# NTT123/vietTTS

Hardware: NVIDIA H100
Metric: audio_samples_per_sec (higher is better)
Workload: dtype f32 (bf16x3 split products on wgmma tensor cores, fp32 accumulate/storage)

## Files before the change

viettts_b200/csrc/tc_conv.cu:

```cuda
#include <cuda_bf16.h>

#include <algorithm>

#include "tc_common.cuh"
#include "vtts_internal.cuh"

namespace {

using namespace tcx;

constexpr int NCWG = 2;
constexpr int NCONS = NCWG * 128;
constexpr int PROD_WARP = NCONS / 32;
constexpr int NCONV = 96;
constexpr int NTHREADS = NCONS + 32 + NCONV;
constexpr int NA = 4;
constexpr int HALO = 64;
constexpr int PAIR_OVERLAP = 16;
constexpr int NQ = 2;
constexpr int NREADERS = (NCONS + NCONV) / 32;

template <int N, int MW, int PAIRF, bool STAGED = false>
struct TcCfg {
  static constexpr int R = 64 * MW * NCWG;
  static constexpr int R_OUT = R - PAIR_OVERLAP;
  static constexpr int RA = R + HALO;
  static constexpr int A_STAGE = RA * 64;
  static constexpr int W_STAGE = N * 64;
  static constexpr int NW = N == 256 ? 4 : 8;
  static constexpr int NCH2 = PAIRF ? N / 16 : 0;
  static constexpr int EPI_NC = N < 128 ? N : 128;
  static constexpr int EPI_LD = EPI_NC + 8;
  static constexpr int EPI_WG = 64 * EPI_LD + N;
  static constexpr int EPI_STAGE = STAGED ? NCWG * EPI_WG * 4 : 0;
  static constexpr int SMEM_BYTES =
      NA * A_STAGE + NW * W_STAGE + NCH2 * A_STAGE + EPI_STAGE + (2 * NA + 2 * NW + 2 * NQ) * 8 + NQ * 4 + 1024;
  static_assert(SMEM_BYTES <= 227 * 1024, "shared memory of one CTA");
};

struct Ring {
  uint32_t s = 0, p = 0;
  template <int NS>
  __device__ __forceinline__ void next() { if (++s == NS) { s = 0; p ^= 1; } }
};

struct Tile {
  int pi, b, tt, ph;
};
__device__ __forceinline__ Tile decode_tile(int t, int nph, int nprob, int tiles_per_row) {
  Tile d;
  d.ph = t % nph; t /= nph;
  d.pi = t % nprob; t /= nprob;
  d.tt = t % tiles_per_row;
  d.b = t / tiles_per_row;
  return d;
}

__device__ __forceinline__ int take_ticket(int* sched, int ntiles) {
  const int t = (int)gridDim.x + atomicAdd(&sched[0], 1);
  if (t < ntiles) return t;
  __threadfence();
  if (atomicAdd(&sched[1], 1) == (int)gridDim.x - 1) {
    atomicExch(&sched[0], 0);
    atomicExch(&sched[1], 0);
  }
  return -1;
}

struct TileQueue {
  int* id;
  uint64_t* full;
  uint64_t* empty;
  Ring r;
  __device__ __forceinline__ void put(int t, int* err, long long& acc) {
    mbar_wait_t(&empty[r.s], r.p ^ 1, err, 6, acc);
    id[r.s] = t;
    mbar_arrive(&full[r.s]);
    r.next<NQ>();
  }
  __device__ __forceinline__ int get(int* err, long long& acc) {
    int t = 0;
    if ((threadIdx.x & 31) == 0) {
      mbar_wait_t(&full[r.s], r.p, err, 6, acc);
      t = id[r.s];
      mbar_arrive(&empty[r.s]);
    }
    r.next<NQ>();
    return __shfl_sync(0xffffffffu, t, 0);
  }
};

template <int RA, bool F16>
__device__ __forceinline__ void convert_chunk(uint8_t* stage, int ct, const float* x0, const float* x1, const float* x2, int ld, int c,
                                              int row_base, int rows, int lo, int valid, int pre_mode, float slope) {
  constexpr int RSTEP = NCONV / 4;
  const int q = ct & 3;
  const int r0 = ct >> 2;
  uint8_t* st = stage + ((q >> 1) * RA) * 16 + (q & 1) * 8;
  const int coff = c * 16 + q * 4;
  constexpr int U = 8;
  for (int rr0 = r0; rr0 < rows; rr0 += RSTEP * U) {
    float4 v[U];
#pragma unroll
    for (int u = 0; u < U; ++u) {
      const int rr = rr0 + u * RSTEP;
      const int t = row_base + rr;
      v[u] = make_float4(0.f, 0.f, 0.f, 0.f);
      if (rr < rows && t >= lo && t < valid) {
        const size_t off = (size_t)t * ld + coff;
        v[u] = ldg_pf256(x0 + off);
        if (pre_mode == 2) {
          const float4 a = ldg_pf256(x1 + off);
          const float4 bb = ldg_pf256(x2 + off);
          v[u].x = ((v[u].x + a.x) + bb.x) / 3.0f;
          v[u].y = ((v[u].y + a.y) + bb.y) / 3.0f;
          v[u].z = ((v[u].z + a.z) + bb.z) / 3.0f;
          v[u].w = ((v[u].w + a.w) + bb.w) / 3.0f;
        }
      }
    }
#pragma unroll
    for (int u = 0; u < U; ++u) {
      const int rr = rr0 + u * RSTEP;
      if (rr < rows) {
        float4 x = v[u];
        if (pre_mode >= 1) {
          x.x = lrelu(x.x, slope); x.y = lrelu(x.y, slope); x.z = lrelu(x.z, slope); x.w = lrelu(x.w, slope);
        }
        if constexpr (F16) {
          *reinterpret_cast<uint2*>(st + (size_t)rr * 16) = f16x4_sat(x);
        } else {
          uint2 hi, lo;
          split4(x, hi, lo);
          *reinterpret_cast<uint2*>(st + (size_t)rr * 16) = hi;
          *reinterpret_cast<uint2*>(st + (size_t)(2 * RA + rr) * 16) = lo;
        }
      }
    }
  }
}

template <int N, int NW, bool F16>
__device__ __forceinline__ void produce_weights(uint8_t* w_st, uint64_t* w_full, uint64_t* w_empty, Ring& rw, const void* wpk, int nch,
                                                int k, int* err, long long& wait_acc) {
  constexpr int WB = F16 ? N * 32 : N * 64;
  const uint8_t* src = reinterpret_cast<const uint8_t*>(wpk);
  for (int i = 0; i < nch * k; ++i) {
    mbar_wait_t(&w_empty[rw.s], rw.p ^ 1, err, 4, wait_acc);
    mbar_expect_tx(&w_full[rw.s], WB);
    bulk_g2s(w_st + rw.s * (N * 64), src + (size_t)i * WB, WB, &w_full[rw.s]);
    rw.next<NW>();
  }
}

template <int N, int MW, int RA, int NW, bool A_FROM_RING, bool A_REGS, bool F16>
__device__ __forceinline__ void consume(float (&acc)[MW][N / 2], int wg, uint32_t a_st_u32, uint64_t* a_full, uint64_t* a_empty, Ring& ra,
                                        uint32_t w_st_u32, uint64_t* w_full, uint64_t* w_empty, Ring& rw, int nch, int k, int dil,
                                        int* err, long long& w_a, long long& w_w) {
  const uint64_t a_tmpl = make_desc(0, RA * 16, 128);
  const uint64_t b_tmpl = make_desc(0, (F16 ? 1 : 2) * N * 16, 128);
  const bool lane0 = (threadIdx.x & 31) == 0;
  int pend_w = -1, pend_a = -1;
  for (int c = 0; c < nch; ++c) {
    uint32_t a_base;
    if constexpr (A_FROM_RING) {
      mbar_wait_t(&a_full[ra.s], ra.p, err, 2, w_a);
      a_base = a_st_u32 + ra.s * (RA * 64);
    } else {
      a_base = a_st_u32 + c * (RA * 64);
    }
    for (int j = 0; j < k; ++j) {
      mbar_wait_t(&w_full[rw.s], rw.p, err, 3, w_w);
      const uint32_t w_base = w_st_u32 + rw.s * (N * 64);
      const uint64_t b_hi = b_tmpl | (uint64_t)(w_base >> 4);
      const uint64_t b_lo = b_tmpl | (uint64_t)((w_base + N * 16) >> 4);
      const uint32_t first = (c | j) != 0 ? 1u : 0u;
      if constexpr (A_REGS) {
        static_assert(!A_FROM_RING && !F16, "register A operand: bf16 planes of the fixed buffer");
        const int lane = threadIdx.x & 31, wl = (threadIdx.x >> 5) & 3;
        uint32_t fa_hi[MW][4], fa_lo[MW][4];
#pragma unroll
        for (int mt = 0; mt < MW; ++mt) {
          const int row = (wg * MW + mt) * 64 + wl * 16 + ((lane >> 3) & 1) * 8 + (lane & 7) + j * dil;
          const uint32_t addr = a_base + ((lane >> 4) * RA + row) * 16;
          ldmatrix_x4(fa_hi[mt], addr);
          ldmatrix_x4(fa_lo[mt], addr + 2 * RA * 16);
        }
        wgmma_fence();
#pragma unroll
        for (int mt = 0; mt < MW; ++mt) {
          wgmma_rs<N>(acc[mt], fa_hi[mt], b_hi, first);
          wgmma_rs<N>(acc[mt], fa_hi[mt], b_lo, 1u);
          wgmma_rs<N>(acc[mt], fa_lo[mt], b_hi, 1u);
        }
        wgmma_commit();
        wgmma_wait<0>();
        if (lane == 0) mbar_arrive(&w_empty[rw.s]);
        rw.next<NW>();
        continue;
      }
      wgmma_fence();
#pragma unroll
      for (int mt = 0; mt < MW; ++mt) {
        const uint32_t row = a_base + ((wg * MW + mt) * 64 + j * dil) * 16;
        const uint64_t a_hi = a_tmpl | (uint64_t)(row >> 4);
        const uint64_t a_lo = a_tmpl | (uint64_t)((row + 2 * RA * 16) >> 4);
        if constexpr (F16) {
          wgmma<N, true>(acc[mt], a_hi, b_hi, first);
        } else {
          wgmma<N>(acc[mt], a_hi, b_hi, first);
          wgmma<N>(acc[mt], a_hi, b_lo, 1u);
          wgmma<N>(acc[mt], a_lo, b_hi, 1u);
        }
      }
      wgmma_commit();
      wgmma_wait<1>();
      if (lane0) {
        if (pend_w >= 0) mbar_arrive(&w_empty[pend_w]);
        if (pend_a >= 0) mbar_arrive(&a_empty[pend_a]);
      }
      pend_w = (int)rw.s;
      pend_a = (A_FROM_RING && j == k - 1) ? (int)ra.s : -1;
      rw.next<NW>();
    }
    if constexpr (A_FROM_RING) ra.next<NA>();
  }
  wgmma_wait<0>();
  if (lane0) {
    if (pend_w >= 0) mbar_arrive(&w_empty[pend_w]);
    if (pend_a >= 0) mbar_arrive(&a_empty[pend_a]);
  }
}

__device__ __forceinline__ void cp_async16(void* smem_dst, const void* gsrc) {
  asm volatile("cp.async.cg.shared.global [%0], [%1], 16;" ::"r"(smem_u32(smem_dst)), "l"(gsrc) : "memory");
}
__device__ __forceinline__ void cp_async_commit() { asm volatile("cp.async.commit_group;" ::: "memory"); }
__device__ __forceinline__ void cp_async_wait_all() { asm volatile("cp.async.wait_all;" ::: "memory"); }

__device__ __forceinline__ void init_barriers(uint64_t* bars, int nw) {
  uint64_t* a_full = bars;
  uint64_t* a_empty = bars + NA;
  uint64_t* w_full = bars + 2 * NA;
  uint64_t* w_empty = bars + 2 * NA + nw;
  uint64_t* q_full = bars + 2 * NA + 2 * nw;
  uint64_t* q_empty = q_full + NQ;
  for (int i = 0; i < NA; ++i) { mbar_init(&a_full[i], NCONV); mbar_init(&a_empty[i], NCONS / 32); }
  for (int i = 0; i < nw; ++i) { mbar_init(&w_full[i], 1); mbar_init(&w_empty[i], NCONS / 32); }
  for (int i = 0; i < NQ; ++i) { mbar_init(&q_full[i], 1); mbar_init(&q_empty[i], NREADERS); }
  asm volatile("fence.mbarrier_init.release.cluster;" ::: "memory");
}

__device__ __forceinline__ TileQueue tile_queue(uint64_t* bars, int nw) {
  uint64_t* q_full = bars + 2 * NA + 2 * nw;
  return TileQueue{reinterpret_cast<int*>(q_full + 2 * NQ), q_full, q_full + NQ, Ring{}};
}

#define PRODUCER_TILES                                                                     \
  TileQueue q = tile_queue(bars, NW);                                                      \
  long long w_q = 0;                                                                       \
  int t_next = blockIdx.x;                                                                 \
  q.put(t_next, L.err, w_q);                                                               \
  auto next_tile = [&]() {                                                                 \
    const int t = t_next;                                                                  \
    if (t >= 0) { t_next = take_ticket(L.sched, L.ntiles); q.put(t_next, L.err, w_q); }    \
    return t;                                                                              \
  };
#define READER_TILES                                                                       \
  TileQueue q = tile_queue(bars, NW);                                                      \
  long long w_q = 0;                                                                       \
  auto next_tile = [&]() { return q.get(L.err, w_q); };

template <int N, int EPI, int MW, bool F16>
__global__ void __launch_bounds__(NTHREADS, 1) tc_conv_kernel(const __grid_constant__ TcLaunch L) {
  using Cfg = TcCfg<N, MW, 0, EPI == 0>;
  constexpr int R = Cfg::R, RA = Cfg::RA, NW = Cfg::NW;
  extern __shared__ uint8_t smem_raw[];
  uint8_t* smem = (uint8_t*)(((uintptr_t)smem_raw + 1023) & ~(uintptr_t)1023);
  uint8_t* a_st = smem;
  uint8_t* w_st = smem + NA * Cfg::A_STAGE;
  float* epi_st = reinterpret_cast<float*>(smem_raw + (w_st + NW * Cfg::W_STAGE - smem_raw));
  uint64_t* bars = reinterpret_cast<uint64_t*>(w_st + NW * Cfg::W_STAGE + Cfg::EPI_STAGE);
  uint64_t* a_full = bars;
  uint64_t* a_empty = bars + NA;
  uint64_t* w_full = bars + 2 * NA;
  uint64_t* w_empty = bars + 2 * NA + NW;

  const int tid = threadIdx.x;
  const int warp = __shfl_sync(0xffffffffu, tid >> 5, 0);
  if (tid == 0) init_barriers(bars, NW);
  __syncthreads();

  const int nch = L.Cin / 16;
  const int nph = L.nphase > 1 ? L.nphase : 1;

  constexpr bool ROW_BOUNDS = EPI == 0;
#define TILE_LOOP_BEGIN                                                           \
  for (int tile; (tile = next_tile()) >= 0;) {                                    \
    const Tile td = decode_tile(tile, nph, L.nprob, L.tiles_per_row);              \
    const int ph = td.ph, b = td.b;                                                 \
    const int tau0 = td.tt * R;                                                    \
    const TcProb& P = L.p[td.pi];                                                  \
    int valid = L.T_rows, in_lo = 0, out_hi = 0;                                  \
    if (ROW_BOUNDS && P.rb) {                                                     \
      in_lo = P.rb[3 * b]; valid = P.rb[3 * b + 1]; out_hi = P.rb[3 * b + 2];     \
      if (tau0 * P.out_stride + P.out_off_ph[ph] >= out_hi) continue;             \
    } else {                                                                      \
      if (L.len) {                                                                \
        const int v = L.len[b] * L.len_mul;                                       \
        valid = v < valid ? v : valid;                                            \
      }                                                                           \
      if (tau0 >= valid) continue;                                                \
    }
#define TILE_LOOP_END }

  if (warp == PROD_WARP) {
    if ((tid & 31) == 0) {
      Ring rw;
      long long w_e = 0;
      PRODUCER_TILES
      TILE_LOOP_BEGIN
        (void)b; (void)tau0; (void)in_lo; (void)valid; (void)out_hi;
        produce_weights<N, NW, F16>(w_st, w_full, w_empty, rw, P.wpk_ph[ph], nch, P.k, L.err, w_e);
      TILE_LOOP_END
      if (L.dbg) L.dbg[(size_t)blockIdx.x * 16 + 4] = w_e;
    }
  } else if (warp > PROD_WARP) {
    const int ct = tid - NCONS - 32;
    Ring ra;
    long long w_ae = 0;
    READER_TILES
    TILE_LOOP_BEGIN
      const int k = P.k, dil = P.dil;
      const size_t in_base = (size_t)b * L.T_rows * L.in_ld;
      const float* x1 = L.pre_mode == 2 ? P.x1 + in_base : nullptr;
      const float* x2 = L.pre_mode == 2 ? P.x2 + in_base : nullptr;
      for (int c = 0; c < nch; ++c) {
        mbar_wait_t(&a_empty[ra.s], ra.p ^ 1, L.err, 5, w_ae);
        convert_chunk<RA, F16>(a_st + ra.s * Cfg::A_STAGE, ct, P.x0 + in_base, x1, x2, L.in_ld, c, tau0 + P.in_off_ph[ph], R + (k - 1) * dil,
                          in_lo, valid, L.pre_mode, L.pre_slope);
        fence_proxy_async();
        mbar_arrive(&a_full[ra.s]);
        ra.next<NA>();
      }
      (void)out_hi;
    TILE_LOOP_END
    if (L.dbg && ct == 0) L.dbg[(size_t)blockIdx.x * 16 + 5] = w_ae;
  } else {
    const int wg = warp >> 2, lane = tid & 31;
    float acc[MW][N / 2];
    Ring ra, rw;
    long long w_a = 0, w_w = 0, t_epi = 0;
    const long long t_begin = clock64();
    const int n_valid = (EPI && L.n_valid > 0) ? L.n_valid : N;
    const int post_act = EPI ? L.post_act : 0;
    constexpr int EPI_NC = Cfg::EPI_NC, EPI_LD = Cfg::EPI_LD, RPS = 128 / (EPI_NC / 4), NQ4 = 64 / RPS;
    float* stg = epi_st + wg * Cfg::EPI_WG;
    float* stg_bias = stg + 64 * EPI_LD;
    const int fr = (warp & 3) * 16 + (lane >> 2), fc = 2 * (lane & 3);
    const int dr = (tid & 127) / (EPI_NC / 4), dq = (tid & 127) % (EPI_NC / 4);
    READER_TILES
    TILE_LOOP_BEGIN
      const size_t out_base = (size_t)b * L.rows_out * L.out_ld;
      const int ostride = P.out_stride, ooff = P.out_off_ph[ph];
      auto row_ok = [&](int tau) { return (ROW_BOUNDS && P.rb) ? tau * ostride + ooff < out_hi : tau < valid; };
      auto fetch_pass = [&](int mt, int nh) {
        if (P.resid) {
          const int blk = tau0 + (wg * MW + mt) * 64;
#pragma unroll
          for (int i = 0; i < NQ4; ++i) {
            const int row = i * RPS + dr, tau = blk + row;
            if (row_ok(tau))
              cp_async16(stg + row * EPI_LD + dq * 4, P.resid + out_base + ((tau * ostride + ooff) * L.out_ld + nh * EPI_NC + dq * 4));
          }
        }
        cp_async_commit();
      };
      auto wait_pass = [&]() {
        cp_async_wait_all();
        named_bar(2 + wg, 128);
      };
      if constexpr (EPI == 0) {
        if ((tid & 127) < N / 4) cp_async16(stg_bias + (tid & 127) * 4, P.bias + (tid & 127) * 4);
        fetch_pass(0, 0);
      }
      consume<N, MW, RA, NW, true, false, F16>(acc, wg, smem_u32(a_st), a_full, a_empty, ra, smem_u32(w_st), w_full, w_empty, rw, nch, P.k,
                                               P.dil, L.err, w_a, w_w);
      const long long t_epi0 = clock64();
      if constexpr (EPI == 0) {
        wait_pass();
#pragma unroll
        for (int mt = 0; mt < MW; ++mt) {
          if (!row_ok(tau0 + (wg * MW + mt) * 64)) break;
#pragma unroll
          for (int nh = 0; nh < N / EPI_NC; ++nh) {
            if (mt + nh > 0 && P.resid) {
              fetch_pass(mt, nh);
              wait_pass();
            }
#pragma unroll
            for (int jn = 0; jn < EPI_NC / 8; ++jn) {
              const int col = jn * 8 + fc, e = (nh * (EPI_NC / 8) + jn) * 4;
              const float2 bi = *reinterpret_cast<const float2*>(stg_bias + nh * EPI_NC + col);
#pragma unroll
              for (int h = 0; h < 2; ++h) {
                float2* s = reinterpret_cast<float2*>(stg + (fr + 8 * h) * EPI_LD + col);
                float2 o = make_float2(acc[mt][e + 2 * h] + bi.x, acc[mt][e + 2 * h + 1] + bi.y);
                if (P.resid) {
                  const float2 r = *s;
                  o.x += r.x; o.y += r.y;
                }
                *s = o;
              }
            }
            named_bar(2 + wg, 128);
            const int blk = tau0 + (wg * MW + mt) * 64;
#pragma unroll
            for (int i = 0; i < NQ4; ++i) {
              const int row = i * RPS + dr, tau = blk + row;
              if (row_ok(tau))
                *reinterpret_cast<float4*>(P.out + out_base + ((tau * ostride + ooff) * L.out_ld + nh * EPI_NC + dq * 4)) =
                    *reinterpret_cast<const float4*>(stg + row * EPI_LD + dq * 4);
            }
            named_bar(2 + wg, 128);
          }
        }
      } else {
        const int row_w = tau0 + wg * MW * 64 + (warp & 3) * 16 + (lane >> 2);
#pragma unroll
        for (int mt = 0; mt < MW; ++mt)
#pragma unroll
          for (int h = 0; h < 2; ++h) {
            const int tau = row_w + mt * 64 + 8 * h;
            if (!row_ok(tau)) continue;
            const size_t orow = out_base + (size_t)(tau * ostride + ooff) * L.out_ld;
#pragma unroll
            for (int jn = 0; jn < N / 8; ++jn) {
              const int col = jn * 8 + 2 * (lane & 3);
              if (col >= n_valid) continue;
              float2 o = make_float2(acc[mt][jn * 4 + 2 * h], acc[mt][jn * 4 + 2 * h + 1]);
              const float2 bi = __ldg(reinterpret_cast<const float2*>(P.bias + col));
              o.x += bi.x; o.y += bi.y;
              if (P.bn_mean) {
                const float2 mu = __ldg(reinterpret_cast<const float2*>(P.bn_mean + col));
                const float2 iv = __ldg(reinterpret_cast<const float2*>(P.bn_inv + col));
                const float2 of = __ldg(reinterpret_cast<const float2*>(P.bn_off + col));
                o.x = (o.x - mu.x) * iv.x + of.x; o.y = (o.y - mu.y) * iv.y + of.y;
              }
              if (post_act == 1) { o.x = tanhf(o.x); o.y = tanhf(o.y); }
              else if (post_act == 2) { o.x = fmaxf(o.x, 0.f); o.y = fmaxf(o.y, 0.f); }
              if (P.resid) {
                const float2 r = __ldg(reinterpret_cast<const float2*>(P.resid + orow + col));
                o.x += r.x; o.y += r.y;
              }
              *reinterpret_cast<float2*>(P.out + orow + col) = o;
            }
          }
      }
      t_epi += clock64() - t_epi0;
    TILE_LOOP_END
    if (L.dbg && tid == 0) {
      long long* d = L.dbg + (size_t)blockIdx.x * 16;
      d[0] = clock64() - t_begin; d[1] = t_epi; d[2] = w_a; d[3] = w_w;
    }
  }
#undef TILE_LOOP_BEGIN
#undef TILE_LOOP_END
}

template <int N, int MW, bool A2_REGS, bool F16>
__global__ void __launch_bounds__(NTHREADS, 1) tc_pair_kernel(const __grid_constant__ TcPairLaunch L) {
  using Cfg = TcCfg<N, MW, 1>;
  constexpr int R = Cfg::R, R_OUT = Cfg::R_OUT, RA = Cfg::RA, NW = Cfg::NW, NCH = N / 16;
  extern __shared__ uint8_t smem_raw[];
  uint8_t* smem = (uint8_t*)(((uintptr_t)smem_raw + 1023) & ~(uintptr_t)1023);
  uint8_t* a_st = smem;
  uint8_t* w_st = smem + NA * Cfg::A_STAGE;
  uint8_t* mid = w_st + NW * Cfg::W_STAGE;
  uint64_t* bars = reinterpret_cast<uint64_t*>(mid + Cfg::NCH2 * Cfg::A_STAGE);
  uint64_t* a_full = bars;
  uint64_t* a_empty = bars + NA;
  uint64_t* w_full = bars + 2 * NA;
  uint64_t* w_empty = bars + 2 * NA + NW;

  const int tid = threadIdx.x;
  const int warp = __shfl_sync(0xffffffffu, tid >> 5, 0);
  if (tid == 0) init_barriers(bars, NW);
  __syncthreads();

#define TILE_LOOP_BEGIN                                                   \
  for (int tile; (tile = next_tile()) >= 0;) {                            \
    const Tile td = decode_tile(tile, 1, L.nprob, L.tiles_per_row);        \
    const int b = td.b;                                                    \
    const int tau0 = td.tt * R_OUT;                                        \
    int valid = L.T_rows;                                                 \
    if (L.len) {                                                          \
      const int v = L.len[b] * L.len_mul;                                 \
      valid = v < valid ? v : valid;                                      \
    }                                                                     \
    if (tau0 >= valid) continue;                                          \
    const TcPairProb& P = L.p[td.pi];                                      \
    const int k = P.k, dil = P.dil, h2 = (k - 1) / 2;
#define TILE_LOOP_END }

  if (warp == PROD_WARP) {
    if ((tid & 31) == 0) {
      Ring rw;
      long long w_e = 0;
      PRODUCER_TILES
      TILE_LOOP_BEGIN
        (void)b; (void)tau0; (void)dil; (void)h2;
        produce_weights<N, NW, F16>(w_st, w_full, w_empty, rw, P.w1pk, NCH, k, L.err, w_e);
        produce_weights<N, NW, F16>(w_st, w_full, w_empty, rw, P.w2pk, NCH, k, L.err, w_e);
      TILE_LOOP_END
    }
  } else if (warp > PROD_WARP) {
    const int ct = tid - NCONS - 32;
    Ring ra;
    long long w_ae = 0;
    READER_TILES
    TILE_LOOP_BEGIN
      const float* x = P.x + (size_t)b * L.T_rows * N;
      const int row_base = tau0 - h2 - (k - 1) * dil / 2;
      for (int c = 0; c < NCH; ++c) {
        mbar_wait_t(&a_empty[ra.s], ra.p ^ 1, L.err, 5, w_ae);
        convert_chunk<RA, F16>(a_st + ra.s * Cfg::A_STAGE, ct, x, nullptr, nullptr, N, c, row_base, R + (k - 1) * dil, 0, valid, 1, L.slope);
        fence_proxy_async();
        mbar_arrive(&a_full[ra.s]);
        ra.next<NA>();
      }
    TILE_LOOP_END
  } else {
    const int wg = warp >> 2, lane = tid & 31;
    float acc[MW][N / 2];
    Ring ra, rw;
    long long w_a = 0, w_w = 0;
    const long long t_begin = clock64();
    const float slope = L.slope;
    READER_TILES
    TILE_LOOP_BEGIN
      consume<N, MW, RA, NW, true, false, F16>(acc, wg, smem_u32(a_st), a_full, a_empty, ra, smem_u32(w_st), w_full, w_empty, rw, NCH, k, dil,
                                               L.err, w_a, w_w);
      const int lr_w = wg * MW * 64 + (warp & 3) * 16 + (lane >> 2);
#pragma unroll
      for (int mt = 0; mt < MW; ++mt)
#pragma unroll
        for (int h = 0; h < 2; ++h) {
          const int lr = lr_w + mt * 64 + 8 * h;
          const int u = tau0 - h2 + lr;
          const bool inside = u >= 0 && u < valid;
#pragma unroll
          for (int jn = 0; jn < N / 8; ++jn) {
            const int col = jn * 8 + 2 * (lane & 3);
            const float2 bi = __ldg(reinterpret_cast<const float2*>(P.b1 + col));
            const float v0 = inside ? lrelu(acc[mt][jn * 4 + 2 * h] + bi.x, slope) : 0.f;
            const float v1 = inside ? lrelu(acc[mt][jn * 4 + 2 * h + 1] + bi.y, slope) : 0.f;
            uint8_t* dst = mid + (col >> 4) * Cfg::A_STAGE + (((col >> 3) & 1) * RA + lr) * 16 + (col & 7) * 2;
            if constexpr (F16) {
              *reinterpret_cast<uint32_t*>(dst) = f16x2_sat(v0, v1);
            } else {
              const __nv_bfloat162 hi = __floats2bfloat162_rn(v0, v1);
              const __nv_bfloat162 lo = __floats2bfloat162_rn(v0 - __low2float(hi), v1 - __high2float(hi));
              *reinterpret_cast<__nv_bfloat162*>(dst) = hi;
              *reinterpret_cast<__nv_bfloat162*>(dst + 2 * RA * 16) = lo;
            }
          }
        }
      fence_proxy_async();
      named_bar(1, NCONS);
      consume<N, MW, RA, NW, false, A2_REGS, F16>(acc, wg, smem_u32(mid), a_full, a_empty, ra, smem_u32(w_st), w_full, w_empty, rw, NCH, k, 1,
                                                  L.err, w_a, w_w);
      named_bar(1, NCONS);
      const float* x = P.x + (size_t)b * L.T_rows * N;
      float* out = P.out + (size_t)b * L.T_rows * N;
#pragma unroll
      for (int mt = 0; mt < MW; ++mt)
#pragma unroll
        for (int h = 0; h < 2; ++h) {
          const int lr = lr_w + mt * 64 + 8 * h;
          const int tau = tau0 + lr;
          if (lr >= R_OUT || tau >= valid) continue;
#pragma unroll
          for (int jn = 0; jn < N / 8; ++jn) {
            const int col = jn * 8 + 2 * (lane & 3);
            const float2 bi = __ldg(reinterpret_cast<const float2*>(P.b2 + col));
            const float2 r = __ldg(reinterpret_cast<const float2*>(x + (size_t)tau * N + col));
            float2 o;
            o.x = acc[mt][jn * 4 + 2 * h] + bi.x + r.x;
            o.y = acc[mt][jn * 4 + 2 * h + 1] + bi.y + r.y;
            *reinterpret_cast<float2*>(out + (size_t)tau * N + col) = o;
          }
        }
    TILE_LOOP_END
    if (L.dbg && tid == 0) {
      long long* d = L.dbg + (size_t)blockIdx.x * 16;
      d[0] = clock64() - t_begin; d[2] = w_a; d[3] = w_w;
    }
  }
#undef TILE_LOOP_BEGIN
#undef TILE_LOOP_END
}

template <bool F16>
__global__ void pack_w_kernel(const float* __restrict__ w, uint16_t* __restrict__ dst, int k, int Cin, int Cout_total, int n0, int N) {
  const size_t total = (size_t)k * Cin * N;
  for (size_t idx = blockIdx.x * (size_t)blockDim.x + threadIdx.x; idx < total; idx += (size_t)gridDim.x * blockDim.x) {
    const int n = idx % N;
    const int i = (idx / N) % Cin;
    const int j = idx / ((size_t)N * Cin);
    const float v = (n0 + n) < Cout_total ? w[((size_t)j * Cin + i) * Cout_total + n0 + n] : 0.f;
    const int c = i / 16, kh = (i % 16) / 8, e = i % 8;
    if constexpr (F16) {
      const size_t blk = ((size_t)c * k + j) * (size_t)(2 * N * 8);
      dst[blk + ((size_t)kh * N + n) * 8 + e] = (uint16_t)(f16x2_sat(v, 0.f) & 0xffffu);
      continue;
    }
    const __nv_bfloat16 hi = __float2bfloat16_rn(v);
    const __nv_bfloat16 lo = __float2bfloat16_rn(v - __bfloat162float(hi));
    const size_t blk = ((size_t)c * k + j) * (size_t)(4 * N * 8);
    dst[blk + ((size_t)(kh * 2 + 0) * N + n) * 8 + e] = __bfloat16_as_ushort(hi);
    dst[blk + ((size_t)(kh * 2 + 1) * N + n) * 8 + e] = __bfloat16_as_ushort(lo);
  }
}

template <int N, int EPI, int MW, bool F16>
int launch_cfg(vtts_ctx* ctx, TcLaunch& L, cudaStream_t st) {
  using Cfg = TcCfg<N, MW, 0, EPI == 0>;
  static bool attr_done_dev[64] = {};
  if (!attr_done_dev[ctx->device & 63]) {
    VTTS_CUDA(cudaFuncSetAttribute(tc_conv_kernel<N, EPI, MW, F16>, cudaFuncAttributeMaxDynamicSharedMemorySize, Cfg::SMEM_BYTES));
    attr_done_dev[ctx->device & 63] = true;
  }
  const int nph = L.nphase > 1 ? L.nphase : 1;
  for (int i = 0; i < L.nprob; ++i) {
    if (nph == 1) {
      L.p[i].wpk_ph[0] = L.p[i].wpk;
      L.p[i].in_off_ph[0] = L.p[i].in_off;
      L.p[i].out_off_ph[0] = L.p[i].out_off;
    }
    if ((L.p[i].k - 1) * L.p[i].dil > HALO) return ctx->fail(VTTS_ERR_BAD_ARG, "tc_conv: halo too large");
  }
  std::stable_sort(L.p, L.p + L.nprob, [](const TcProb& a, const TcProb& b) { return a.k > b.k; });
  L.tiles_per_row = ((L.tile_rows > 0 ? L.tile_rows : L.T_rows) + Cfg::R - 1) / Cfg::R;
  L.ntiles = L.nprob * L.tiles_per_row * L.B * nph;
  const int grid = L.ntiles < ctx->sm_count ? L.ntiles : ctx->sm_count;
  tc_conv_kernel<N, EPI, MW, F16><<<grid, NTHREADS, Cfg::SMEM_BYTES, st>>>(L);
  ctx->launches++;
  VTTS_CUDA(cudaGetLastError());
  return VTTS_OK;
}

template <int N>
int launch_n(vtts_ctx* ctx, TcLaunch& L, cudaStream_t st) {
  constexpr int MW = N >= 256 ? 1 : (N == 128 ? 2 : 4);
  bool generic = L.post_act != 0 || (L.n_valid > 0 && L.n_valid < N);
  bool rb = false;
  for (int i = 0; i < L.nprob; ++i) {
    generic |= L.p[i].bn_mean != nullptr;
    rb |= L.p[i].rb != nullptr;
  }
  if (rb && generic) return ctx->fail(VTTS_ERR_BAD_ARG, "tc_conv: per-row bounds use the plain epilogue");
  if (!generic) {
    if ((int64_t)L.rows_out * L.out_ld > INT32_MAX) return ctx->fail(VTTS_ERR_BAD_ARG, "tc_conv: %d output rows of %d", L.rows_out, L.out_ld);
    bool aligned = L.out_ld % 4 == 0;
    for (int i = 0; i < L.nprob; ++i) aligned &= (((uintptr_t)L.p[i].out | (uintptr_t)L.p[i].resid | (uintptr_t)L.p[i].bias) & 15) == 0;
    if (!aligned) return ctx->fail(VTTS_ERR_BAD_ARG, "tc_conv: the plain epilogue needs 16-byte aligned out / resid rows and bias (out_ld %d)", L.out_ld);
  }
  if (L.nphase > 4) return ctx->fail(VTTS_ERR_BAD_ARG, "tc_conv: %d phases", L.nphase);
  if (L.nphase > 1 && generic) return ctx->fail(VTTS_ERR_BAD_ARG, "tc_conv: multi-phase tiles use the plain epilogue");
  if (L.f16 && generic) return ctx->fail(VTTS_ERR_BAD_ARG, "tc_conv: fp16 operands use the plain epilogue");
  if (L.f16) return launch_cfg<N, 0, MW, true>(ctx, L, st);
  return generic ? launch_cfg<N, 1, MW, false>(ctx, L, st) : launch_cfg<N, 0, MW, false>(ctx, L, st);
}

template <int N, int MW, bool A2_REGS, bool F16 = false>
int launch_pair(vtts_ctx* ctx, TcPairLaunch& L, cudaStream_t st) {
  using Cfg = TcCfg<N, MW, 1>;
  static bool attr_done_dev[64] = {};
  if (!attr_done_dev[ctx->device & 63]) {
    VTTS_CUDA(cudaFuncSetAttribute(tc_pair_kernel<N, MW, A2_REGS, F16>, cudaFuncAttributeMaxDynamicSharedMemorySize, Cfg::SMEM_BYTES));
    attr_done_dev[ctx->device & 63] = true;
  }
  for (int i = 0; i < L.nprob; ++i)
    if (L.p[i].k - 1 > PAIR_OVERLAP || (L.p[i].k - 1) * L.p[i].dil > HALO) return ctx->fail(VTTS_ERR_BAD_ARG, "tc_pair: halo too large");
  std::stable_sort(L.p, L.p + L.nprob, [](const TcPairProb& a, const TcPairProb& b) { return a.k > b.k; });
  L.tiles_per_row = (L.T_rows + Cfg::R_OUT - 1) / Cfg::R_OUT;
  L.ntiles = L.nprob * L.tiles_per_row * L.B;
  const int grid = L.ntiles < ctx->sm_count ? L.ntiles : ctx->sm_count;
  tc_pair_kernel<N, MW, A2_REGS, F16><<<grid, NTHREADS, Cfg::SMEM_BYTES, st>>>(L);
  ctx->launches++;
  VTTS_CUDA(cudaGetLastError());
  return VTTS_OK;
}

}

size_t vtts_tc_packed_elems(int k, int Cin, int N, bool f16) { return (size_t)k * Cin * N * (f16 ? 1 : 2); }

int vtts_tc_pack_weights(vtts_ctx* ctx, const float* w, void* dst, int k, int Cin, int Cout_total, int n0, int N, bool f16) {
  if (f16) pack_w_kernel<true><<<256, 256>>>(w, reinterpret_cast<uint16_t*>(dst), k, Cin, Cout_total, n0, N);
  else pack_w_kernel<false><<<256, 256>>>(w, reinterpret_cast<uint16_t*>(dst), k, Cin, Cout_total, n0, N);
  VTTS_CUDA(cudaGetLastError());
  return VTTS_OK;
}

int vtts_tc_tile_n(int Cout) { return Cout <= 32 ? 32 : (Cout <= 64 ? 64 : (Cout <= 128 ? 128 : 256)); }

size_t vtts_tc_conv_packed_bytes(int k, int Cin, int Cout, bool f16) {
  const int N = vtts_tc_tile_n(Cout), nt = (Cout + N - 1) / N;
  return ((vtts_tc_packed_elems(k, Cin, N, f16) * 2 + 255) & ~size_t(255)) * nt;
}

int vtts_tc_pack_conv(vtts_ctx* ctx, const float* w, int k, int Cin, int Cout, bool f16, char*& cursor, std::vector<void*>& out) {
  const int N = vtts_tc_tile_n(Cout), nt = (Cout + N - 1) / N;
  for (int t = 0; t < nt; ++t) {
    int rc = vtts_tc_pack_weights(ctx, w, cursor, k, Cin, Cout, t * N, N, f16);
    if (rc) return rc;
    out.push_back(cursor);
    cursor += (vtts_tc_packed_elems(k, Cin, N, f16) * 2 + 255) & ~size_t(255);
  }
  return VTTS_OK;
}

int vtts_conv_dispatch(vtts_ctx* ctx, const ConvLaunch& L, void* const* wpk, cudaStream_t st) {
  if (ctx->precision == VTTS_PRECISION_FP32 || wpk == nullptr) return vtts_launch_conv(ctx, L, st);
  const int N = vtts_tc_tile_n(L.Cout), nt = (L.Cout + N - 1) / N;
  TcLaunch TL;
  auto reset = [&]() {
    memset(&TL, 0, sizeof(TL));
    TL.Cin = L.Cin; TL.N = N; TL.in_ld = L.Cin; TL.out_ld = L.Cout; TL.B = L.B; TL.T_rows = L.T_rows; TL.rows_out = L.rows_out;
    TL.len = L.len; TL.len_mul = L.len_mul; TL.pre_mode = L.pre_mode; TL.pre_slope = L.pre_slope; TL.post_act = L.post_act;
    TL.n_valid = (L.Cout % N) ? (L.Cout % N) : N;
  };
  reset();
  for (int pass = 0; pass < 2; ++pass) {
    const bool partial = pass == 1;
    if (partial && (L.Cout % N) == 0) break;
    reset();
    TL.n_valid = partial ? (L.Cout % N) : N;
    for (int pi = 0; pi < L.nprob; ++pi) {
      const ConvProb& cp = L.p[pi];
      for (int t = 0; t < nt; ++t) {
        const bool is_partial = (t == nt - 1) && (L.Cout % N) != 0;
        if (is_partial != partial) continue;
        const int n0 = t * N;
        TcProb q;
        memset(&q, 0, sizeof(q));
        q.x0 = cp.x0; q.x1 = cp.x1; q.x2 = cp.x2;
        q.wpk = wpk[pi * nt + t];
        q.bias = cp.bias + n0;
        q.resid = cp.resid ? cp.resid + n0 : nullptr;
        if (cp.bn_mean) { q.bn_mean = cp.bn_mean + n0; q.bn_inv = cp.bn_inv + n0; q.bn_off = cp.bn_off + n0; }
        q.out = cp.out + n0;
        q.k = cp.k; q.dil = cp.dil; q.in_off = cp.in_off; q.out_stride = cp.out_stride; q.out_off = cp.out_off;
        TL.p[TL.nprob++] = q;
        if (TL.nprob == 8) {
          int rc = vtts_launch_tc_conv(ctx, TL, st);
          if (rc) return rc;
          TL.nprob = 0;
        }
      }
    }
    if (TL.nprob > 0) {
      int rc = vtts_launch_tc_conv(ctx, TL, st);
      if (rc) return rc;
    }
  }
  return VTTS_OK;
}

int vtts_launch_tc_conv(vtts_ctx* ctx, TcLaunch& L, cudaStream_t st) {
  if (L.nprob < 1 || L.nprob > 8) return ctx->fail(VTTS_ERR_BAD_ARG, "tc_conv: nprob %d", L.nprob);
  if (L.Cin % 16 != 0) return ctx->fail(VTTS_ERR_BAD_ARG, "tc_conv: Cin %d", L.Cin);
  for (int i = 0; i < L.nprob; ++i)
    if (L.p[i].k < 1) return ctx->fail(VTTS_ERR_BAD_ARG, "tc_conv: k");
  L.sched = ctx->d_tc_sched;
  L.err = ctx->d_err;
  L.dbg = ctx->tc_dbg_on ? ctx->d_tc_dbg : nullptr;
  switch (L.N) {
    case 256: return launch_n<256>(ctx, L, st);
    case 128: return launch_n<128>(ctx, L, st);
    case 64: return launch_n<64>(ctx, L, st);
    case 32: return launch_n<32>(ctx, L, st);
    default: return ctx->fail(VTTS_ERR_BAD_ARG, "tc_conv: N %d unsupported", L.N);
  }
}

int vtts_launch_tc_pair(vtts_ctx* ctx, TcPairLaunch& L, cudaStream_t st) {
  if (L.nprob < 1 || L.nprob > 3) return ctx->fail(VTTS_ERR_BAD_ARG, "tc_pair: nprob %d", L.nprob);
  for (int i = 0; i < L.nprob; ++i)
    if (L.p[i].k < 1 || L.p[i].x == L.p[i].out) return ctx->fail(VTTS_ERR_BAD_ARG, "tc_pair: bad problem %d", i);
  L.sched = ctx->d_tc_sched;
  L.err = ctx->d_err;
  L.dbg = ctx->tc_dbg_on ? ctx->d_tc_dbg : nullptr;
  if (L.N != 32 && L.N != 64) return ctx->fail(VTTS_ERR_BAD_ARG, "tc_pair: C %d unsupported (32 or 64)", L.N);
  if (L.f16) {
    if (ctx->pair_ts != 2) return ctx->fail(VTTS_ERR_BAD_ARG, "tc_pair: fp16 operands exist for the default pair form (256-row tiles) only, not form %d", ctx->pair_ts);
    return L.N == 64 ? launch_pair<64, 2, false, true>(ctx, L, st) : launch_pair<32, 2, false, true>(ctx, L, st);
  }
  if (ctx->pair_ts == 1) return L.N == 64 ? launch_pair<64, 2, true>(ctx, L, st) : launch_pair<32, 2, true>(ctx, L, st);
  if (ctx->pair_ts == 0) return L.N == 64 ? launch_pair<64, 1, false>(ctx, L, st) : launch_pair<32, 1, false>(ctx, L, st);
  return L.N == 64 ? launch_pair<64, 2, false>(ctx, L, st) : launch_pair<32, 2, false>(ctx, L, st);
}
```

viettts_b200/engine.py:

```python
from __future__ import annotations

import ctypes as C
import threading
from typing import NamedTuple

import numpy as np

from . import _lib, config, weights

DROPOUT_OFF, DROPOUT_MASK, DROPOUT_SEED, DROPOUT_REFERENCE = 0, 1, 2, 3


def _chunk_seed(seed: int, chunk: int) -> int:
    return (int(seed) ^ (chunk * 0x9E3779B97F4A7C15)) & 0xFFFFFFFFFFFFFFFF


def _rng_seed(rng, *others) -> int:
    if any(o is not None for o in others):
        raise ValueError("rng= selects the reference's own mask stream; it cannot be combined with masks= or seed=")
    w = np.asarray(rng).ravel()
    if w.size != 2 or not np.issubdtype(w.dtype, np.integer):
        raise ValueError(f"rng must hold exactly two integer words (the checkpoint's uint32[2] rng), got {np.asarray(rng).shape}")
    return ((int(w[0]) & 0xFFFFFFFF) << 32) | (int(w[1]) & 0xFFFFFFFF)
PRECISION_FP32, PRECISION_BF16X3, PRECISION_FP16 = 0, 1, 2
PRECISIONS = {"fp32": PRECISION_FP32, "bf16x3": PRECISION_BF16X3, "fp16": PRECISION_FP16}
MAX_ACOUSTIC_ROWS = 128


def resample_ratio(in_rate: int, out_rate: int):
    from math import gcd
    in_rate, out_rate = int(in_rate), int(out_rate)
    if in_rate <= 0 or out_rate <= 0:
        raise ValueError(f"sample rates must be positive, got {in_rate} -> {out_rate}")
    g = gcd(in_rate, out_rate)
    return out_rate // g, in_rate // g


def resample_length(n: int, in_rate: int, out_rate: int) -> int:
    up, down = resample_ratio(in_rate, out_rate)
    return -(-int(n) * up // down)


DENOISE_BINS = config.N_FFT // 2 + 1
DENOISE_BIAS_FRAMES = 88


def _strength(s) -> float:
    s = float(s)
    if not (np.isfinite(s) and s >= 0):
        raise ValueError(f"denoise strength must be finite and >= 0, got {s}")
    return s


MAX_SEMITONES = 12.0


def _semitones(v, n: int) -> np.ndarray:
    a = np.asarray(v, np.float32)
    a = np.full(n, a, np.float32) if a.ndim == 0 else np.ascontiguousarray(a.reshape(-1), np.float32)
    if a.shape != (n,):
        raise ValueError(f"semitones: one value or one per row ({n}), got {np.shape(v)}")
    if not (np.all(np.isfinite(a)) and np.all(np.abs(a) <= MAX_SEMITONES)):
        raise ValueError(f"semitones must be finite and lie in [-12, 12], got {v}")
    return a


def _ptr(a):
    if a is None:
        return None
    if isinstance(a, np.ndarray):
        return a.ctypes.data
    return a.data_ptr()


def _np(a, dtype, shape=None, what="array"):
    a = np.ascontiguousarray(np.asarray(a), dtype=dtype)
    if shape is not None and tuple(a.shape) != tuple(shape):
        raise ValueError(f"{what}: expected shape {tuple(shape)}, got {tuple(a.shape)}")
    return a


class Engine:

    def __init__(self, device: int = 0):
        self.lib = _lib.load()
        self.device = int(device)
        h = _lib.c_ctx()
        rc = self.lib.vtts_create(self.device, C.byref(h))
        if rc != 0:
            msg = self.lib.vtts_last_error(None)
            raise _lib.VttsError(rc, msg.decode() if msg else "?")
        self.h = h
        self._hifigan_key = None
        self._acoustic_key = None
        self._duration_key = None
        self._mel_loaded = False
        self._denoise_bias = None

    def close(self):
        if getattr(self, "h", None):
            self.lib.vtts_destroy(self.h)
            self.h = None

    def __del__(self):
        try:
            self.close()
        except Exception:
            pass

    def _ck(self, rc):
        _lib.check(self.h, rc)

    def device_info(self) -> dict:
        sm, ma, mi, hb = C.c_int(), C.c_int(), C.c_int(), C.c_int64()
        self._ck(self.lib.vtts_device_info(self.h, C.byref(sm), C.byref(ma), C.byref(mi), C.byref(hb)))
        return dict(sm_count=sm.value, cc=(ma.value, mi.value), hbm_bytes=hb.value)

    def launch_count(self) -> int:
        return int(self.lib.vtts_launch_count(self.h))

    def last_stage_ms(self, stage: int) -> float:
        ms = C.c_float()
        self._ck(self.lib.vtts_last_stage_ms(self.h, stage, C.byref(ms)))
        return float(ms.value)

    def set_precision(self, mode) -> None:
        m = PRECISIONS.get(mode, mode)
        self._ck(self.lib.vtts_set_precision(self.h, int(m)))
        self._denoise_bias = None

    def debug_conv1d(self, precision, x_t, w_t, bias_t, k, dil, pre_slope=1.0, resid_t=None, len_t=None):
        import torch
        B, T, Cin = x_t.shape
        Cout = w_t.shape[2]
        out = torch.empty((B, T, Cout), dtype=torch.float32, device=x_t.device)
        m = PRECISIONS.get(precision, precision)
        self._ck(self.lib.vtts_debug_conv1d(self.h, int(m), _ptr(x_t), _ptr(w_t), _ptr(bias_t), _ptr(resid_t), _ptr(len_t),
                                            B, T, Cin, Cout, int(k), int(dil), float(pre_slope), _ptr(out)))
        return out

    POST_ACTS = {"none": 0, "tanh": 1, "relu": 2}

    def debug_conv_dispatch(self, precision, xs, ws, biases, k, dil=1, bns=None, resids=None, post_act="none", len_t=None, outs=None):
        import torch
        n = len(xs)
        B, T, Cin = xs[0].shape
        Cout = ws[0].shape[2]
        if outs is None:
            outs = [torch.empty((B, T, Cout), dtype=torch.float32, device=xs[0].device) for _ in range(n)]

        def arr(ts):
            return None if ts is None else (C.c_void_p * n)(*[_ptr(t) for t in ts])

        m = PRECISIONS.get(precision, precision)
        self._ck(self.lib.vtts_debug_conv_dispatch(self.h, int(m), n, arr(xs), arr(ws), arr(biases), arr(bns), arr(resids), arr(outs),
                                                   _ptr(len_t), B, T, Cin, Cout, int(k), int(dil), self.POST_ACTS[post_act]))
        return outs

    def debug_pair(self, x_t, w1_t, b1_t, w2_t, b2_t, k, dil, slope=0.1, len_t=None):
        import torch
        B, T, Cc = x_t.shape
        out = torch.empty_like(x_t)
        self._ck(self.lib.vtts_debug_pair(self.h, _ptr(x_t), _ptr(w1_t), _ptr(b1_t), _ptr(w2_t), _ptr(b2_t), _ptr(len_t),
                                          B, T, Cc, int(k), int(dil), float(slope), _ptr(out)))
        return out

    HIFIGAN_LAYERS = 18

    def debug_hifigan_layer(self, layer, xs, outs, n_frames_t=None, T=None):
        scale = [1, 1, 8, 64, 128] + [8] * 3 + [64] * 3 + [128] * 3 + [256] * 3 + [256]
        B, rows = xs[0].shape[:2]
        if T is None:
            T = rows // scale[layer]
        arr = lambda ts: (C.c_void_p * len(ts))(*[_ptr(t) for t in ts])
        self._ck(self.lib.vtts_debug_hifigan_layer(self.h, int(layer), arr(xs), arr(outs), _ptr(n_frames_t), int(B), int(T)))
        return outs

    PAIR_KERNELS = {"smem": 0, "tmem": 1, "smem2": 2}

    def set_fused_pairs(self, on: bool, kind: str | None = None):
        flags = 0x200 | ((1 if on else 0) << 10)
        if kind is not None:
            flags |= 0x800 | (self.PAIR_KERNELS[kind] << 12)
        self._ck(self.lib.vtts_debug_tc_stats(self.h, flags, None))
        self._denoise_bias = None

    def tc_stats(self, enable=True):
        out = np.zeros((256, 16), np.int64)
        self._ck(self.lib.vtts_debug_tc_stats(self.h, 1 if enable else 0, _ptr(out)))
        return out

    SUBSTAGES = {1: "acoustic.encoder", 2: "acoustic.upsample", 3: "acoustic.cond_gemm", 4: "acoustic.decoder_scan",
                 5: "acoustic.projection", 6: "acoustic.postnet", 9: "hifigan.conv_pre", 10: "hifigan.stage0", 11: "hifigan.stage1",
                 12: "hifigan.stage2", 13: "hifigan.stage3", 14: "hifigan.conv_post", 17: "teacher.encoder_upsample",
                 18: "teacher.prenet_hoisted_gemm", 19: "teacher.zoneout_scan", 20: "teacher.projection_postnet"}

    def substages(self, enable=True) -> dict:
        out = np.zeros(24, np.float32)
        self._ck(self.lib.vtts_debug_substages(self.h, 1 if enable else 0, _ptr(out)))
        return {name: float(out[i]) for i, name in self.SUBSTAGES.items() if out[i] > 0}

    def _load(self, fn, pack, src):
        blob = pack(src) if isinstance(src, dict) else src
        n = int(blob.size if isinstance(blob, np.ndarray) else blob.numel())
        if isinstance(blob, np.ndarray):
            blob = _np(blob, np.float32)
        self._ck(fn(self.h, _ptr(blob), n))

    def load_hifigan(self, params, key=None):
        self._load(self.lib.vtts_load_hifigan, weights.pack_hifigan, params)
        self._hifigan_key = key if key is not None else object()
        self._denoise_bias = None

    def load_acoustic(self, ckpt, key=None):
        self._load(self.lib.vtts_load_acoustic, weights.pack_acoustic, ckpt)
        self._acoustic_key = key if key is not None else object()

    def load_duration(self, ckpt, key=None):
        self._load(self.lib.vtts_load_duration, weights.pack_duration, ckpt)
        self._duration_key = key if key is not None else object()

    def broadcast_weights(self, nccl_comm, root: int, is_root: bool, stream=None):
        self._ck(self.lib.vtts_broadcast_weights(self.h, nccl_comm, int(root), 1 if is_root else 0, stream))
        self._denoise_bias = None
        if not is_root:
            self._hifigan_key = self._acoustic_key = self._duration_key = object()

    def load_mel_filterbank(self, fb=None):
        fb = _np(weights.mel_filterbank() if fb is None else fb, np.float32, (config.MEL_DIM, config.N_FFT // 2 + 1), "filterbank")
        self._ck(self.lib.vtts_load_mel_filterbank(self.h, _ptr(fb), fb.shape[0], fb.shape[1]))
        self._mel_loaded = True

    def mel2wave(self, mel, n_frames=None, out=None) -> np.ndarray:
        mel = _np(mel, np.float32)
        if mel.ndim != 3 or mel.shape[2] != config.MEL_DIM:
            raise ValueError(f"mel must be [B,T,{config.MEL_DIM}], got {mel.shape}")
        B, T, _ = mel.shape
        nf = None if n_frames is None else _np(n_frames, np.int32, (B,), "n_frames")
        if out is not None and (out.shape != (B, T * config.HOP) or out.dtype != np.float32 or not out.flags.c_contiguous):
            raise ValueError(f"out must be C-contiguous float32 {(B, T * config.HOP)}")
        wav = out if out is not None else np.empty((B, T * config.HOP), np.float32)
        self._ck(self.lib.vtts_mel2wave_host(self.h, _ptr(mel), _ptr(nf), B, T, _ptr(wav)))
        return wav

    STREAM_HALO = 16

    def mel2wave_stream(self, mel, chunk_frames: int = 32, halo: int | None = None):
        mel = _np(mel, np.float32)
        if mel.ndim == 3:
            if mel.shape[0] != 1:
                raise ValueError("mel2wave_stream takes one utterance ([T,80] or [1,T,80])")
            mel = mel[0]
        if mel.ndim != 2 or mel.shape[1] != config.MEL_DIM:
            raise ValueError(f"mel must be [T,{config.MEL_DIM}], got {mel.shape}")
        halo = self.STREAM_HALO if halo is None else int(halo)
        if chunk_frames < 1 or halo < 0:
            raise ValueError("chunk_frames >= 1 and halo >= 0 required")
        T = mel.shape[0]
        for t0 in range(0, T, chunk_frames):
            t1 = min(T, t0 + chunk_frames)
            a, b = max(0, t0 - halo), min(T, t1 + halo)
            wav = self.mel2wave(mel[None, a:b])[0]
            yield wav[(t0 - a) * config.HOP: (t1 - a) * config.HOP]

    def open_vocoder_stream(self, max_streams: int, max_chunk_frames: int) -> "VocoderStream":
        return VocoderStream(self, max_streams, max_chunk_frames)

    def open_acoustic_stream(self, max_streams: int, max_chunk_frames: int, max_frames: int, max_tokens: int, seed=None, rng=None,
                             masks: bool = False) -> "AcousticStream":
        return AcousticStream(self, max_streams, max_chunk_frames, max_frames, max_tokens, seed=seed, rng=rng, masks=masks)

    def open_tts_stream(self, max_streams: int, max_chunk_frames: int, max_frames: int, max_tokens: int = 1024, seed=None,
                        rng=None, output_rate=None, denoise=None, meter=False, semitones=None) -> "TtsStream":
        return TtsStream(self, max_streams, max_chunk_frames, max_frames, max_tokens, seed=seed, rng=rng, output_rate=output_rate,
                         denoise=denoise, meter=meter, semitones=semitones)

    def tts_plan(self, tokens, lengths=None, silence_duration=-1.0):
        tokens = _np(tokens, np.int32)
        if tokens.ndim != 2:
            raise ValueError("tokens must be [B,L]")
        B, L = tokens.shape
        lens = None if lengths is None else _np(lengths, np.int32, (B,), "lengths")
        sec = np.empty((B, L), np.float32)
        frames = np.empty((B, L), np.float32)
        nf = np.empty(B, np.int32)
        ne = np.empty(B, np.int32)
        self._ck(self.lib.vtts_tts_plan(self.h, _ptr(tokens), _ptr(lens), B, L, float(silence_duration), _ptr(sec), _ptr(frames),
                                        _ptr(nf), _ptr(ne)))
        return sec, frames, nf, ne

    def get_precision(self) -> int:
        return int(self.lib.vtts_get_precision(self.h))

    def _acoustic_args(self, tokens, dur_frames, lengths, n_frames, masks, seed, rng=None):
        ref_seed = None if rng is None else _rng_seed(rng, masks, seed)
        tokens = _np(tokens, np.int32)
        if tokens.ndim != 2:
            raise ValueError("tokens must be [B,L]")
        B, L = tokens.shape
        dur = _np(dur_frames, np.float32, (B, L), "durations")
        lens = None if lengths is None else _np(lengths, np.int32, (B,), "lengths")
        if n_frames is None:
            nf = np.array([int(np.sum(dur[b, : (L if lens is None else lens[b])], dtype=np.float32)) for b in range(B)], np.int32)
        else:
            nf = _np(n_frames, np.int32, (B,), "n_frames")
        N = int(nf.max())
        if N < 1:
            raise ValueError("durations sum to less than one frame")
        if ref_seed is not None:
            return tokens, dur, lens, nf, N, None, DROPOUT_REFERENCE, ref_seed
        if masks is not None:
            mode = DROPOUT_MASK
            masks = _np(masks, np.uint8)
            if masks.shape[0] != B or masks.shape[1] < N or masks.shape[2:] != (2, config.PRENET_DIM):
                raise ValueError(f"masks must be uint8 [B,>=N,2,256], got {masks.shape}")
# ... 1081 lines not shown
```

Baseline: 54.23 million.

## Stage pair-kernel residual epilogue through swizzled smem and enlarge C=32 tiles

```diff
diff --git a/viettts_b200/csrc/tc_conv.cu b/viettts_b200/csrc/tc_conv.cu
--- a/viettts_b200/csrc/tc_conv.cu
+++ b/viettts_b200/csrc/tc_conv.cu
@@ -14,7 +14,6 @@
 constexpr int PROD_WARP = NCONS / 32;
 constexpr int NCONV = 96;
 constexpr int NTHREADS = NCONS + 32 + NCONV;
-constexpr int NA = 4;
 constexpr int HALO = 64;
 constexpr int PAIR_OVERLAP = 16;
 constexpr int NQ = 2;
@@ -26,6 +25,7 @@
   static constexpr int R_OUT = R - PAIR_OVERLAP;
   static constexpr int RA = R + HALO;
   static constexpr int A_STAGE = RA * 64;
+  static constexpr int NA = PAIRF && R == 512 ? 3 : 4;
   static constexpr int W_STAGE = N * 64;
   static constexpr int NW = N == 256 ? 4 : 8;
   static constexpr int NCH2 = PAIRF ? N / 16 : 0;
@@ -153,7 +153,7 @@
   }
 }
 
-template <int N, int MW, int RA, int NW, bool A_FROM_RING, bool A_REGS, bool F16>
+template <int N, int MW, int RA, int NA, int NW, bool A_FROM_RING, bool A_REGS, bool F16>
 __device__ __forceinline__ void consume(float (&acc)[MW][N / 2], int wg, uint32_t a_st_u32, uint64_t* a_full, uint64_t* a_empty, Ring& ra,
                                         uint32_t w_st_u32, uint64_t* w_full, uint64_t* w_empty, Ring& rw, int nch, int k, int dil,
                                         int* err, long long& w_a, long long& w_w) {
@@ -238,6 +238,7 @@
 __device__ __forceinline__ void cp_async_commit() { asm volatile("cp.async.commit_group;" ::: "memory"); }
 __device__ __forceinline__ void cp_async_wait_all() { asm volatile("cp.async.wait_all;" ::: "memory"); }
 
+template <int NA>
 __device__ __forceinline__ void init_barriers(uint64_t* bars, int nw) {
   uint64_t* a_full = bars;
   uint64_t* a_empty = bars + NA;
@@ -251,13 +252,14 @@
   asm volatile("fence.mbarrier_init.release.cluster;" ::: "memory");
 }
 
+template <int NA>
 __device__ __forceinline__ TileQueue tile_queue(uint64_t* bars, int nw) {
   uint64_t* q_full = bars + 2 * NA + 2 * nw;
   return TileQueue{reinterpret_cast<int*>(q_full + 2 * NQ), q_full, q_full + NQ, Ring{}};
 }
 
 #define PRODUCER_TILES                                                                     \
-  TileQueue q = tile_queue(bars, NW);                                                      \
+  TileQueue q = tile_queue<NA>(bars, NW);                                                  \
   long long w_q = 0;                                                                       \
   int t_next = blockIdx.x;                                                                 \
   q.put(t_next, L.err, w_q);                                                               \
@@ -267,14 +269,14 @@
     return t;                                                                              \
   };
 #define READER_TILES                                                                       \
-  TileQueue q = tile_queue(bars, NW);                                                      \
+  TileQueue q = tile_queue<NA>(bars, NW);                                                  \
   long long w_q = 0;                                                                       \
   auto next_tile = [&]() { return q.get(L.err, w_q); };
 
 template <int N, int EPI, int MW, bool F16>
 __global__ void __launch_bounds__(NTHREADS, 1) tc_conv_kernel(const __grid_constant__ TcLaunch L) {
   using Cfg = TcCfg<N, MW, 0, EPI == 0>;
-  constexpr int R = Cfg::R, RA = Cfg::RA, NW = Cfg::NW;
+  constexpr int R = Cfg::R, RA = Cfg::RA, NA = Cfg::NA, NW = Cfg::NW;
   extern __shared__ uint8_t smem_raw[];
   uint8_t* smem = (uint8_t*)(((uintptr_t)smem_raw + 1023) & ~(uintptr_t)1023);
   uint8_t* a_st = smem;
@@ -288,7 +290,7 @@
 
   const int tid = threadIdx.x;
   const int warp = __shfl_sync(0xffffffffu, tid >> 5, 0);
-  if (tid == 0) init_barriers(bars, NW);
+  if (tid == 0) init_barriers<NA>(bars, NW);
   __syncthreads();
 
   const int nch = L.Cin / 16;
@@ -384,7 +386,7 @@
         if ((tid & 127) < N / 4) cp_async16(stg_bias + (tid & 127) * 4, P.bias + (tid & 127) * 4);
         fetch_pass(0, 0);
       }
-      consume<N, MW, RA, NW, true, false, F16>(acc, wg, smem_u32(a_st), a_full, a_empty, ra, smem_u32(w_st), w_full, w_empty, rw, nch, P.k,
+      consume<N, MW, RA, NA, NW, true, false, F16>(acc, wg, smem_u32(a_st), a_full, a_empty, ra, smem_u32(w_st), w_full, w_empty, rw, nch, P.k,
                                                P.dil, L.err, w_a, w_w);
       const long long t_epi0 = clock64();
       if constexpr (EPI == 0) {
@@ -471,12 +473,15 @@
 template <int N, int MW, bool A2_REGS, bool F16>
 __global__ void __launch_bounds__(NTHREADS, 1) tc_pair_kernel(const __grid_constant__ TcPairLaunch L) {
   using Cfg = TcCfg<N, MW, 1>;
-  constexpr int R = Cfg::R, R_OUT = Cfg::R_OUT, RA = Cfg::RA, NW = Cfg::NW, NCH = N / 16;
+  constexpr int R = Cfg::R, R_OUT = Cfg::R_OUT, RA = Cfg::RA, NA = Cfg::NA, NW = Cfg::NW, NCH = N / 16;
   extern __shared__ uint8_t smem_raw[];
   uint8_t* smem = (uint8_t*)(((uintptr_t)smem_raw + 1023) & ~(uintptr_t)1023);
   uint8_t* a_st = smem;
   uint8_t* w_st = smem + NA * Cfg::A_STAGE;
   uint8_t* mid = w_st + NW * Cfg::W_STAGE;
+  float* const stg = reinterpret_cast<float*>(smem_raw + (mid - smem_raw));
+  static_assert(R * N * 4 <= Cfg::NCH2 * Cfg::A_STAGE, "the staged rows fit in the intermediate");
+  auto staged_at = [](int lr, int col) { return lr * N + (((col >> 2) ^ ((lr & 3) << 1)) << 2) + (col & 3); };
   uint64_t* bars = reinterpret_cast<uint64_t*>(mid + Cfg::NCH2 * Cfg::A_STAGE);
   uint64_t* a_full = bars;
   uint64_t* a_empty = bars + NA;
@@ -485,7 +490,7 @@
 
   const int tid = threadIdx.x;
   const int warp = __shfl_sync(0xffffffffu, tid >> 5, 0);
-  if (tid == 0) init_barriers(bars, NW);
+  if (tid == 0) init_barriers<NA>(bars, NW);
   __syncthreads();
 
 #define TILE_LOOP_BEGIN                                                   \
@@ -534,13 +539,19 @@
     const int wg = warp >> 2, lane = tid & 31;
     float acc[MW][N / 2];
     Ring ra, rw;
-    long long w_a = 0, w_w = 0;
+    long long w_a = 0, w_w = 0, t_epi = 0, t_mid = 0;
     const long long t_begin = clock64();
     const float slope = L.slope;
+    constexpr int RPS = 128 / (N / 4);
+    const int sr = (tid & 127) / (N / 4), sq = (tid & 127) % (N / 4);
+    const int lr0 = wg * MW * 64;
     READER_TILES
     TILE_LOOP_BEGIN
-      consume<N, MW, RA, NW, true, false, F16>(acc, wg, smem_u32(a_st), a_full, a_empty, ra, smem_u32(w_st), w_full, w_empty, rw, NCH, k, dil,
-                                               L.err, w_a, w_w);
+      auto row_ok = [&](int lr) { return lr < R_OUT && tau0 + lr < valid; };
+      consume<N, MW, RA, NA, NW, true, false, F16>(acc, wg, smem_u32(a_st), a_full, a_empty, ra, smem_u32(w_st), w_full, w_empty, rw, NCH, k,
+                                                   dil, L.err, w_a, w_w);
+      const long long t_mid0 = clock64();
+      named_bar(1, NCONS);
       const int lr_w = wg * MW * 64 + (warp & 3) * 16 + (lane >> 2);
 #pragma unroll
       for (int mt = 0; mt < MW; ++mt)
@@ -568,33 +579,52 @@
         }
       fence_proxy_async();
       named_bar(1, NCONS);
-      consume<N, MW, RA, NW, false, A2_REGS, F16>(acc, wg, smem_u32(mid), a_full, a_empty, ra, smem_u32(w_st), w_full, w_empty, rw, NCH, k, 1,
-                                                  L.err, w_a, w_w);
+      t_mid += clock64() - t_mid0;
+      consume<N, MW, RA, NA, NW, false, A2_REGS, F16>(acc, wg, smem_u32(mid), a_full, a_empty, ra, smem_u32(w_st), w_full, w_empty, rw, NCH,
+                                                      k, 1, L.err, w_a, w_w);
+      const long long t_epi0 = clock64();
       named_bar(1, NCONS);
-      const float* x = P.x + (size_t)b * L.T_rows * N;
-      float* out = P.out + (size_t)b * L.T_rows * N;
-#pragma unroll
-      for (int mt = 0; mt < MW; ++mt)
-#pragma unroll
-        for (int h = 0; h < 2; ++h) {
-          const int lr = lr_w + mt * 64 + 8 * h;
-          const int tau = tau0 + lr;
-          if (lr >= R_OUT || tau >= valid) continue;
-#pragma unroll
-          for (int jn = 0; jn < N / 8; ++jn) {
-            const int col = jn * 8 + 2 * (lane & 3);
-            const float2 bi = __ldg(reinterpret_cast<const float2*>(P.b2 + col));
-            const float2 r = __ldg(reinterpret_cast<const float2*>(x + (size_t)tau * N + col));
-            float2 o;
-            o.x = acc[mt][jn * 4 + 2 * h] + bi.x + r.x;
-            o.y = acc[mt][jn * 4 + 2 * h + 1] + bi.y + r.y;
-            *reinterpret_cast<float2*>(out + (size_t)tau * N + col) = o;
+      if (row_ok(lr0)) {
+        const float* x = P.x + (size_t)b * L.T_rows * N;
+        float* out = P.out + (size_t)b * L.T_rows * N;
+#pragma unroll 4
+        for (int i = 0; i < MW * 64 / RPS; ++i) {
+          const int lr = lr0 + i * RPS + sr;
+          if (row_ok(lr)) cp_async16(stg + staged_at(lr, sq * 4), x + (size_t)(tau0 + lr) * N + sq * 4);
+        }
+        cp_async_commit();
+        cp_async_wait_all();
+        named_bar(2 + wg, 128);
+#pragma unroll
+        for (int mt = 0; mt < MW; ++mt)
+#pragma unroll
+          for (int h = 0; h < 2; ++h) {
+            const int lr = lr_w + mt * 64 + 8 * h;
+#pragma unroll
+            for (int jn = 0; jn < N / 8; ++jn) {
+              const int col = jn * 8 + 2 * (lane & 3);
+              const float2 bi = __ldg(reinterpret_cast<const float2*>(P.b2 + col));
+              float2* sp = reinterpret_cast<float2*>(stg + staged_at(lr, col));
+              const float2 r = *sp;
+              float2 o;
+              o.x = acc[mt][jn * 4 + 2 * h] + bi.x + r.x;
+              o.y = acc[mt][jn * 4 + 2 * h + 1] + bi.y + r.y;
+              *sp = o;
+            }
           }
-        }
+        named_bar(2 + wg, 128);
+#pragma unroll 4
+        for (int i = 0; i < MW * 64 / RPS; ++i) {
+          const int lr = lr0 + i * RPS + sr;
+          if (row_ok(lr))
+            *reinterpret_cast<float4*>(out + (size_t)(tau0 + lr) * N + sq * 4) = *reinterpret_cast<const float4*>(stg + staged_at(lr, sq * 4));
+        }
+      }
+      t_epi += clock64() - t_epi0;
     TILE_LOOP_END
     if (L.dbg && tid == 0) {
       long long* d = L.dbg + (size_t)blockIdx.x * 16;
-      d[0] = clock64() - t_begin; d[2] = w_a; d[3] = w_w;
+      d[0] = clock64() - t_begin; d[1] = t_epi; d[2] = w_a; d[3] = w_w; d[6] = t_mid;
     }
   }
 #undef TILE_LOOP_BEGIN
@@ -795,10 +825,10 @@
   L.dbg = ctx->tc_dbg_on ? ctx->d_tc_dbg : nullptr;
   if (L.N != 32 && L.N != 64) return ctx->fail(VTTS_ERR_BAD_ARG, "tc_pair: C %d unsupported (32 or 64)", L.N);
   if (L.f16) {
-    if (ctx->pair_ts != 2) return ctx->fail(VTTS_ERR_BAD_ARG, "tc_pair: fp16 operands exist for the default pair form (256-row tiles) only, not form %d", ctx->pair_ts);
-    return L.N == 64 ? launch_pair<64, 2, false, true>(ctx, L, st) : launch_pair<32, 2, false, true>(ctx, L, st);
+    if (ctx->pair_ts != 2) return ctx->fail(VTTS_ERR_BAD_ARG, "tc_pair: fp16 operands exist for the default pair form only, not form %d", ctx->pair_ts);
+    return L.N == 64 ? launch_pair<64, 2, false, true>(ctx, L, st) : launch_pair<32, 4, false, true>(ctx, L, st);
   }
   if (ctx->pair_ts == 1) return L.N == 64 ? launch_pair<64, 2, true>(ctx, L, st) : launch_pair<32, 2, true>(ctx, L, st);
   if (ctx->pair_ts == 0) return L.N == 64 ? launch_pair<64, 1, false>(ctx, L, st) : launch_pair<32, 1, false>(ctx, L, st);
-  return L.N == 64 ? launch_pair<64, 2, false>(ctx, L, st) : launch_pair<32, 2, false>(ctx, L, st);
-}
+  return L.N == 64 ? launch_pair<64, 2, false>(ctx, L, st) : launch_pair<32, 4, false>(ctx, L, st);
+}
diff --git a/viettts_b200/engine.py b/viettts_b200/engine.py
--- a/viettts_b200/engine.py
+++ b/viettts_b200/engine.py
@@ -157,10 +157,10 @@
                                                    _ptr(len_t), B, T, Cin, Cout, int(k), int(dil), self.POST_ACTS[post_act]))
         return outs
 
-    def debug_pair(self, x_t, w1_t, b1_t, w2_t, b2_t, k, dil, slope=0.1, len_t=None):
+    def debug_pair(self, x_t, w1_t, b1_t, w2_t, b2_t, k, dil, slope=0.1, len_t=None, out_t=None):
         import torch
         B, T, Cc = x_t.shape
-        out = torch.empty_like(x_t)
+        out = torch.empty_like(x_t) if out_t is None else out_t
         self._ck(self.lib.vtts_debug_pair(self.h, _ptr(x_t), _ptr(w1_t), _ptr(b1_t), _ptr(w2_t), _ptr(b2_t), _ptr(len_t),
                                           B, T, Cc, int(k), int(dil), float(slope), _ptr(out)))
         return out
```

New measurement: 55.39 million (median of 6 runs). +2.1%, better.
